# owensgroup/sparsify.me

Measured on AMD Instinct MI355X. Metric: effective GF/s (2:4 spmma vs dense gemm) on ResNet-50 layer shapes, higher is better.
Workload: dtype f16

## Files before the change

sparsify.me_amd/csrc/spmma_f16_fused.hip:

```cpp
#include "select24.h"
#include "spmma_args.h"

namespace sm {

constexpr int MAXG = 8;
struct FusedArgs {
  const half_t* A[MAXG];
  const half_t* B[MAXG];
  half_t* C[MAXG];
  size_t sA, sB, sC;
  int Mrows, N, K, lda;
  int batch, tiles_m, tiles_n;
  int ngroup;
  float alpha, beta;
  const half_t* const* dAp;
  const half_t* const* dBp;
  half_t* const* dCp;
};

struct FusedArgsEpi : FusedArgs {
  EpiArgs e;
};
template <bool EPI> struct FusedArgsSel { typedef FusedArgs type; };
template <> struct FusedArgsSel<true> { typedef FusedArgsEpi type; };
// ... 800 lines not shown
      for (; kt0 + 2 * PF < nkt; kt0 += PF) {
#pragma unroll
        for (int u = 0; u < PF; ++u) step(kt0 + u, ra[(u + 1) % PF], true, true);
      }
    } else {
#pragma unroll
      for (int s = 0; s < PF; ++s)
        if (s < nkt) load_a(s, ra[s]);
      write_stage(0, ra[0]);
      if (PF < nkt) load_a(PF, ra[0]);
    }
    for (; kt0 < nkt; kt0 += PF) {
#pragma unroll
      for (int u = 0; u < PF; ++u) {
        const int kt = kt0 + u;
        if (kt < nkt) step(kt, ra[(u + 1) % PF], kt + 1 < nkt, kt + 1 + PF < nkt);
      }
    }
  } else {
    int cb = 0;
    BTileDma<BN, NBW> bd;
    int nb = NSB - 1;
    if (NLB == 0) {
      bd.setup(p.B[grp] + (size_t)b * p.sB, p.N, n0, wave, lane, BRING);
#pragma unroll
      for (int s = 0; s < NSB - 1; ++s)
        if (s < nkt) bd.issue(smem, s, (unsigned)(s * SB));
    }
    for (int kt = 0; kt < nkt; ++kt) {
      if (NLB == 0) {
        if (kt + NSB - 2 < nkt) wait_dma_and_barrier<(NSB - 2) * B_WI>();
        else wait_dma_and_barrier<0>();
        if (kt + NSB - 1 < nkt) {
          bd.issue(smem, kt + NSB - 1, (unsigned)(nb * SB));
          nb = nb + 1 == NSB ? 0 : nb + 1;
        }
      } else {
        wait_dma_and_barrier<0>();
      }
      const char* As = smem + (kt & 1) * ASTG;
      const char* Ms = As + SA;
      const char* Bs = smem + BRING + cb * SB;
      smfmac_stage<FM, FN, BF>(As, Ms, Bs, wm * TM, wn * TN, lane, acc);
      cb = cb + 1 == NSB ? 0 : cb + 1;
    }
  }
  __syncthreads();

  if constexpr (EPI) store_c_tile_epi<BM, BN, FM, FN, 64 * NW, BF>(smem, C, p.e.R + (size_t)b * p.e.sR, p.e, eb, acc, wave < (unsigned)NC, wm * TM, wn * TN, m0, n0, p.Mrows, p.N, p.alpha, p.beta, tid);
  else store_c_tile<BM, BN, FM, FN, 64 * NW, BF>(smem, C, acc, wave < (unsigned)NC, wm * TM, wn * TN, m0, n0, p.Mrows, p.N, p.alpha, p.beta, tid);
}

template <int BN, int WM, int WN, int NLB, int PF, int NSB, bool BF = false, bool ANT = true, bool EPI = false>
static int launch_fused_wide(const typename FusedArgsSel<EPI>::type& a0, hipStream_t st) {
  typename FusedArgsSel<EPI>::type a = a0;
  a.tiles_m = (a.Mrows + 127) / 128;
  a.tiles_n = (a.N + BN - 1) / BN;
  const size_t nwg = (size_t)a.tiles_m * a.tiles_n * a.batch * a.ngroup;
  constexpr size_t lds_main = 2 * (size_t)128 * 72 + (size_t)NSB * 64 * BN * 2;
  constexpr size_t lds_epi = (size_t)128 * (BN * 2 + 16);
  constexpr size_t lds = lds_main > lds_epi ? lds_main : lds_epi;
  return launch_grid<&spmma_f16_fused_wide_kernel<BN, WM, WN, NLB, PF, NSB, BF, ANT, EPI>>(nwg, 64 * (WM * WN + 4 + NLB), lds, lds, st, "sm_spmma_fused_f16",
                                                                                          "spmma_f16_fused_wide_kernel", a);
}

template <int BN, int WM, int WN, int NLB, int PF, int NSB, bool BF = false>
__global__ __launch_bounds__(64 * (WM * WN + 4 + NLB)) void spmma_f16_fused_widep_kernel(const FusedArgs p, const unsigned total) {
  constexpr int BM = 128, NLA = 4, NC = WM * WN;
  static_assert(NLB > 0 && PF >= 1 && PF <= 3 && NSB >= 2 && NSB <= 4, "pipeline depths");
  constexpr int TM = BM / WM, TN = BN / WN, FM = TM / 16, FN = TN / 16;
  static_assert(TN == 128 && TM == 32, "epilogue patch geometry");
  constexpr int SA = BM * 64, SM_ = BM * 8, ASTG = SA + SM_, SB = 64 * BN * 2;
  constexpr int BRING = 2 * ASTG;
  constexpr int B_N = BN / 8, B_WI = B_N / NLB;
  static_assert(B_N % NLB == 0 && (NSB - 2) * B_WI <= 63, "B tile vs loader waves");
  constexpr int WPITCH = 64 * 2 + 8, WPATCH = TM * WPITCH;
  constexpr int CPATCH = BRING + NSB * SB;
  extern __shared__ __attribute__((aligned(16))) char smem[];

  const unsigned tid = threadIdx.x, lane = tid & 63u;
  const unsigned wave = __builtin_amdgcn_readfirstlane(tid >> 6);
  const unsigned tiles = (unsigned)p.tiles_m * (unsigned)p.tiles_n;
  const int nkt = p.K / 64;
  const unsigned my_tiles = (total - blockIdx.x + gridDim.x - 1u) / gridDim.x;
  const int S = (int)my_tiles * nkt;

  struct Tile {
    unsigned grp, b;
    int m0, n0;
  };
  auto tile_of = [&](unsigned j) {
    Tile t;
    const unsigned lid = xcd_remap(blockIdx.x + j * gridDim.x, total);
    const unsigned gb = lid / tiles, trem = lid - gb * tiles;
    t.grp = gb / (unsigned)p.batch;
    t.b = gb - t.grp * (unsigned)p.batch;
    const unsigned tile_m = trem / (unsigned)p.tiles_n, tile_n = trem - tile_m * (unsigned)p.tiles_n;
    t.m0 = (int)tile_m * BM;
    t.n0 = (int)tile_n * BN;
    return t;
  };

  if (wave >= (unsigned)(NC + NLA)) {
    BTileDma<BN, NLB> bd;
    unsigned ij = 0;
    int ikt = 0, nb = 0;
    {
      const Tile t = tile_of(0);
      bd.setup(p.B[t.grp] + (size_t)t.b * p.sB, p.N, t.n0, wave - (NC + NLA), lane, BRING);
    }
    auto issue = [&]() {
      bd.issue(smem, ikt, (unsigned)(nb * SB));
      nb = nb + 1 == NSB ? 0 : nb + 1;
      if (++ikt == nkt) {
        ikt = 0;
        if (++ij < my_tiles) {
          const Tile t = tile_of(ij);
          bd.setup(p.B[t.grp] + (size_t)t.b * p.sB, p.N, t.n0, wave - (NC + NLA), lane, BRING);
        }
      }
    };
#pragma unroll
    for (int s = 0; s < NSB - 1; ++s)
      if (s < S) issue();
    for (int g = 0; g < S; ++g) {
      if (g + NSB - 2 < S) wait_dma_and_barrier<(NSB - 2) * B_WI>();
      else wait_dma_and_barrier<0>();
      if (g + NSB - 1 < S) issue();
    }
  } else if (wave >= (unsigned)NC) {
    const unsigned lw = wave - NC;
    const unsigned c8 = lane & 7u;
    const half_t* a_src[4];
    unsigned a_val_off[4], a_meta_off[4];
#pragma unroll
    for (int i = 0; i < 4; ++i) {
      const unsigned row = 8u * (4u * lw + i) + (lane >> 3);
      a_val_off[i] = row * 64u + 16u * ((c8 >> 1) ^ a64_swz(row)) + 8u * (c8 & 1u);
      a_meta_off[i] = SA + row * 8u + c8;
    }
    const int mlast = p.Mrows - 1;
    auto point_at = [&](unsigned j) {
      const Tile t = tile_of(j);
      const half_t* A = p.A[t.grp] + (size_t)t.b * p.sA;
#pragma unroll
      for (int i = 0; i < 4; ++i) {
        const unsigned row = 8u * (4u * lw + i) + (lane >> 3);
        int gr = t.m0 + (int)row;
        gr = gr < mlast ? gr : mlast;
        a_src[i] = A + (size_t)gr * p.lda + 8u * c8;
      }
    };
    point_at(0);
    unsigned lj = 0;
    int lkt = 0;
    u4 ra[PF][4];
    auto load_a = [&](u4 (&dst)[4]) {
#pragma unroll
      for (int i = 0; i < 4; ++i) dst[i] = __builtin_nontemporal_load(reinterpret_cast<const u4*>(a_src[i] + (size_t)lkt * 64));
      __builtin_amdgcn_sched_barrier(0);
      if (++lkt == nkt) {
        lkt = 0;
        if (++lj < my_tiles) point_at(lj);
      }
    };
    auto write_stage = [&](int g, const u4 (&src)[4]) {
      char* sb = smem + (g & 1) * ASTG;
#pragma unroll
      for (int i = 0; i < 4; ++i) {
        uint32_t k0, k1, n0, n1;
        strip_select_f16(src[i][0], src[i][1], k0, n0);
        strip_select_f16(src[i][2], src[i][3], k1, n1);
        *reinterpret_cast<u2*>(sb + a_val_off[i]) = u2{k0, k1};
        *reinterpret_cast<unsigned char*>(sb + a_meta_off[i]) = (unsigned char)(n0 | (n1 << 4));
      }
    };
    auto step = [&](int g, u4 (&rr)[4], bool write, bool load) {
      asm volatile("s_waitcnt lgkmcnt(0)\n\ts_barrier" ::: "memory");
      __builtin_amdgcn_sched_barrier(0);
      if (write) write_stage(g + 1, rr);
      if (load) load_a(rr);
      __builtin_amdgcn_sched_barrier(0);
    };
    int g0 = 0;
    if (S > 2 * PF) {
#pragma unroll
      for (int s = 0; s < PF; ++s) load_a(ra[s]);
      write_stage(0, ra[0]);
      load_a(ra[0]);
      for (; g0 + 2 * PF < S; g0 += PF) {
#pragma unroll
        for (int u = 0; u < PF; ++u) step(g0 + u, ra[(u + 1) % PF], true, true);
      }
    } else {
#pragma unroll
      for (int s = 0; s < PF; ++s)
        if (s < S) load_a(ra[s]);
      write_stage(0, ra[0]);
      if (PF < S) load_a(ra[0]);
    }
    for (; g0 < S; g0 += PF) {
#pragma unroll
      for (int u = 0; u < PF; ++u) {
        const int g = g0 + u;
        if (g < S) step(g, ra[(u + 1) % PF], g + 1 < S, g + 1 + PF < S);
      }
    }
  } else {
    const unsigned g4 = lane >> 4, r = lane & 15u;
    const unsigned wm = wave / WN, wn = wave % WN;
    char* const patch = smem + CPATCH + wave * WPATCH;
    f4 acc[FM][FN];
#pragma unroll
    for (int i = 0; i < FM; ++i)
#pragma unroll
      for (int j = 0; j < FN; ++j) acc[i][j] = f4{0.f, 0.f, 0.f, 0.f};
    int cb = 0, kt = 0;
    unsigned cj = 0;
    Tile t = tile_of(0);
    for (int g = 0; g < S; ++g) {
      asm volatile("s_barrier" ::: "memory");
      const char* As = smem + (g & 1) * ASTG;
      smfmac_stage<FM, FN, BF>(As, As + SA, smem + BRING + cb * SB, wm * TM, wn * TN, lane, acc);
      cb = cb + 1 == NSB ? 0 : cb + 1;
      if (++kt == nkt) {
        half_t* C = p.C[t.grp] + (size_t)t.b * p.sC;
        const bool c_vec = (reinterpret_cast<uintptr_t>(C) & 15u) == 0 && (p.N % 8 == 0);
        if (p.beta == 0.0f && c_vec) {
#pragma unroll
          for (int h = 0; h < 2; ++h) {
#pragma unroll
            for (int i = 0; i < FM; ++i)
#pragma unroll
              for (int j = 0; j < FN / 2; ++j) {
                const unsigned lr = i * 16 + 4u * g4, lc = j * 16 + r;
#pragma unroll
                for (int q = 0; q < 4; ++q)
                  *reinterpret_cast<half_t*>(patch + (lr + q) * WPITCH + lc * 2) = to_elt<BF>(p.alpha * acc[i][h * (FN / 2) + j][q]);
              }
            asm volatile("s_waitcnt lgkmcnt(0)" ::: "memory");
            const int gc = t.n0 + (int)(wn * TN) + 64 * h + 8 * (int)(lane & 7u);
#pragma unroll
            for (int s8 = 0; s8 < TM / 8; ++s8) {
              const unsigned lr = 8u * s8 + (lane >> 3);
              const int gr = t.m0 + (int)(wm * TM + lr);
              if (gr < p.Mrows && gc < p.N) {
                const u2 lo = *reinterpret_cast<const u2*>(patch + lr * WPITCH + 16u * (lane & 7u));
                const u2 hi = *reinterpret_cast<const u2*>(patch + lr * WPITCH + 16u * (lane & 7u) + 8u);
                __builtin_nontemporal_store(u4{lo[0], lo[1], hi[0], hi[1]}, reinterpret_cast<u4*>(C + (size_t)gr * p.N + gc));
              }
            }
            asm volatile("s_waitcnt lgkmcnt(0)" ::: "memory");
          }
        } else {
#pragma unroll
          for (int i = 0; i < FM; ++i)
#pragma unroll
            for (int j = 0; j < FN; ++j) {
              const int gc = t.n0 + (int)(wn * TN + j * 16 + r);
              if (gc >= p.N) continue;
#pragma unroll
              for (int q = 0; q < 4; ++q) {
                const int gr = t.m0 + (int)(wm * TM + i * 16 + 4u * g4) + q;
                if (gr >= p.Mrows) continue;
                half_t* dst = C + (size_t)gr * p.N + gc;
                float v = p.alpha * acc[i][j][q];
                if (p.beta != 0.0f) v += p.beta * to_f32<BF>(*dst);
                *dst = to_elt<BF>(v);
              }
            }
        }
#pragma unroll
        for (int i = 0; i < FM; ++i)
#pragma unroll
          for (int j = 0; j < FN; ++j) acc[i][j] = f4{0.f, 0.f, 0.f, 0.f};
        kt = 0;
        if (++cj < my_tiles) t = tile_of(cj);
      }
    }
  }
}

template <int BN, int WM, int WN, int NLB, int PF, int NSB, bool BF = false>
static int launch_fused_widep(const FusedArgs& a0, hipStream_t st) {
  FusedArgs a = a0;
  a.tiles_m = (a.Mrows + 127) / 128;
  a.tiles_n = (a.N + BN - 1) / BN;
  const size_t nt = (size_t)a.tiles_m * a.tiles_n * a.batch * a.ngroup;
  if (nt == 0) return SM_STATUS_SUCCESS;
  if (nt > 0x7fffffffu) {
    set_error("sm_spmma_fused_f16: grid too large");
    return SM_STATUS_NOT_SUPPORTED;
  }
  constexpr size_t lds = 2 * (size_t)128 * 72 + (size_t)NSB * 64 * BN * 2 + (size_t)(WM * WN) * 32 * (64 * 2 + 8);
  static_assert(lds > 64 * 1024 && lds <= 160 * 1024, "LDS budget of the persistent wide kernel (always opted in)");
  size_t cus = (size_t)device_cu_count();
  cus -= cus % 8;
  if (cus == 0) cus = 8;
  return launch_grid<&spmma_f16_fused_widep_kernel<BN, WM, WN, NLB, PF, NSB, BF>>(nt <= cus ? nt : cus, 64 * (WM * WN + 4 + NLB), lds, lds, st, "sm_spmma_fused_f16",
                                                                                 "spmma_f16_fused_widep_kernel", a, (unsigned)nt);
}

constexpr int astat_waves_per_simd(int nwaves) { return nwaves == 16 ? 4 : (2 * nwaves + 3) / 4; }
template <int NSB, bool BF = false, int NLA = 4, int NLB = 4, int PR = 32>
__global__ __launch_bounds__(64 * (8 + NLA + NLB), astat_waves_per_simd(8 + NLA + NLB)) void spmma_f16_fused_astat_kernel(const FusedArgs p, int nsplit, int tiles_per_split) {
  constexpr int BM = 128, BN = 128, WM = 4, WN = 2, NC = 8;
  constexpr int NW = NC + NLA + NLB, RPL = (16 + NW - 1) / NW, KTM = 8 / RPL;
  static_assert(NW <= 16 && RPL <= 2 && (PR == 32 || PR == 16 || PR == 8), "launch bounds, phase-1 registers, patch passes");
  constexpr int TM = BM / WM, TN = BN / WN, FM = TM / 16, FN = TN / 16;
  constexpr int SA = BM * 64, SM_ = BM * 8, ASTG = SA + SM_, SB = 64 * BN * 2;
  constexpr int B_N = BN / 8, B_WI = B_N / NLB;
  static_assert((NSB - 2) * B_WI <= 63, "vmcnt range");
  constexpr int WPITCH = TN * 2 + 8, WPATCH = PR * WPITCH;
  static_assert(NLA != 0 || (PR == 16 ? 3 : 4) * ASTG + NSB * SB + NC * WPATCH <= 80 * 1024, "two workgroups per CU: 80 KiB each (astat_pair_lds_bytes)");
  extern __shared__ __attribute__((aligned(16))) char smem[];

  const unsigned tid = threadIdx.x, lane = tid & 63u;
  const unsigned wave = __builtin_amdgcn_readfirstlane(tid >> 6);
  const int nkt = p.K / 64;
  const unsigned per_batch = (unsigned)p.tiles_m * (unsigned)nsplit;
  const unsigned lid = xcd_remap(blockIdx.x, gridDim.x);
  const unsigned gb = lid / per_batch, trem = lid - gb * per_batch;
  const unsigned grp = gb / (unsigned)p.batch, b = gb - grp * (unsigned)p.batch;
  const unsigned tile_m = trem / (unsigned)nsplit, split = trem - tile_m * (unsigned)nsplit;
  const int m0 = (int)tile_m * BM;
  const int nt0 = (int)split * tiles_per_split;
  const int nt1 = nt0 + tiles_per_split < p.tiles_n ? nt0 + tiles_per_split : p.tiles_n;
  const int T = (nt1 - nt0) * nkt;
  char* const Bring = smem + nkt * ASTG;
  char* const Cpatch = Bring + NSB * SB;
  half_t* C = p.C[grp] + (size_t)b * p.sC;

  const bool is_b = wave >= (unsigned)(NC + NLA);
  const unsigned lwb = is_b ? wave - (NC + NLA) : 0u;
  const char* Bb = reinterpret_cast<const char*>(p.B[grp] + (size_t)b * p.sB);
  unsigned b_kr[B_WI], b_col[B_WI], b_dst[B_WI];
  auto b_lanes = [&](unsigned ln) {
#pragma unroll
    for (int i = 0; i < B_WI; ++i) {
      const unsigned j = lwb + (unsigned)NLB * i, panel = j >> 3, grp = j & 7u, kr = 8u * grp + (ln >> 3);
      b_kr[i] = kr;
      b_col[i] = 64u * panel + 8u * ((ln & 7u) ^ b_swz(kr));
      b_dst[i] = panel * 8192u + grp * 1024u;
    }
  };
  b_lanes(lane);
  const size_t row_bytes = (size_t)p.N * 2;
  int i_nt = nt0, i_kt = 0, i_buf = 0;
  auto issue_b = [&]() {
#pragma unroll
    for (int i = 0; i < B_WI; ++i) {
      int gc = i_nt * BN + (int)b_col[i];
      gc = gc <= p.N - 8 ? gc : p.N - 8;
      const char* src = Bb + (size_t)(i_kt * 64 + (int)b_kr[i]) * row_bytes + (size_t)gc * 2;
      __builtin_amdgcn_global_load_lds((gptr_t*)src, (lptr_t*)(Bring + i_buf * SB + b_dst[i]), 16, 0, 0);
    }
    i_buf = i_buf + 1 == NSB ? 0 : i_buf + 1;
    if (++i_kt == nkt) { i_kt = 0; ++i_nt; }
  };
  if (is_b) {
#pragma unroll
    for (int s = 0; s < NSB - 1; ++s)
      if (s < T) issue_b();
  }

  {
    const half_t* A = p.A[grp] + (size_t)b * p.sA;
    const unsigned c8 = lane & 7u;
    u4 ra[RPL][KTM];
#pragma unroll
    for (int h = 0; h < RPL; ++h) {
      const unsigned rg = wave + (unsigned)(NW * h);
      if (RPL == 1 || rg < 16u) {
        int gr = m0 + (int)(8u * rg + (lane >> 3));
        gr = gr < p.Mrows - 1 ? gr : p.Mrows - 1;
        const half_t* a_src = A + (size_t)gr * p.lda + 8u * c8;
#pragma unroll
        for (int s = 0; s < KTM; ++s)
          if (s < nkt) ra[h][s] = __builtin_nontemporal_load(reinterpret_cast<const u4*>(a_src + (size_t)s * 64));
      }
    }
#pragma unroll
    for (int h = 0; h < RPL; ++h) {
      const unsigned rg = wave + (unsigned)(NW * h);
      if (RPL == 1 || rg < 16u) {
        const unsigned row = 8u * rg + (lane >> 3);
        const unsigned a_val_off = row * 64u + 16u * ((c8 >> 1) ^ a64_swz(row)) + 8u * (c8 & 1u);
        const unsigned a_meta_off = SA + row * 8u + c8;
#pragma unroll
        for (int s = 0; s < KTM; ++s)
          if (s < nkt) {
            uint32_t k0, k1, n0, n1;
            strip_select_f16(ra[h][s][0], ra[h][s][1], k0, n0);
            strip_select_f16(ra[h][s][2], ra[h][s][3], k1, n1);
            char* sb = smem + s * ASTG;
            *reinterpret_cast<u2*>(sb + a_val_off) = u2{k0, k1};
            *reinterpret_cast<unsigned char*>(sb + a_meta_off) = (unsigned char)(n0 | (n1 << 4));
          }
      }
    }
  }
  if constexpr (RPL > 1) {
    unsigned ln = lane;
    asm volatile("" : "+v"(ln));
    b_lanes(ln);
  }
  __syncthreads();
  if (wave >= (unsigned)NC && !is_b) {
    for (int it = 0; it < T; ++it) asm volatile("s_barrier" ::: "memory");
    return;
  }

  if (is_b) {
    for (int it = 0; it < T; ++it) {
      if (it + NSB - 2 < T) wait_dma_and_barrier<(NSB - 2) * B_WI>();
      else wait_dma_and_barrier<0>();
      if (it + NSB - 1 < T) issue_b();
    }
  } else {
    const unsigned g = lane >> 4, r = lane & 15u;
    const unsigned wm = wave / WN, wn = wave % WN;
    char* const patch = Cpatch + wave * WPATCH;
    f4 acc[FM][FN];
#pragma unroll
    for (int i = 0; i < FM; ++i)
#pragma unroll
      for (int j = 0; j < FN; ++j) acc[i][j] = f4{0.f, 0.f, 0.f, 0.f};
    int cb = 0, kt = 0, nt = nt0;
    for (int it = 0; it < T; ++it) {
      asm volatile("s_barrier" ::: "memory");
      const char* As = smem + kt * ASTG;
      const char* Ms = As + SA;
      const char* Bs = Bring + cb * SB;
      smfmac_stage<FM, FN, BF>(As, Ms, Bs, wm * TM, wn * TN, lane, acc);
      cb = cb + 1 == NSB ? 0 : cb + 1;
      if (++kt == nkt) {
        if constexpr (PR == TM) {
          const int gc = nt * BN + (int)(wn * TN) + 8 * (int)(lane & 7u);
#pragma unroll
          for (int i = 0; i < FM; ++i)
#pragma unroll
            for (int j = 0; j < FN; ++j) {
              const unsigned lr = i * 16 + 4u * g, lc = j * 16 + r;
#pragma unroll
              for (int q = 0; q < 4; ++q) {
                *reinterpret_cast<half_t*>(patch + (lr + q) * WPITCH + lc * 2) = to_elt<BF>(p.alpha * acc[i][j][q]);
                acc[i][j][q] = 0.f;
              }
            }
          asm volatile("s_waitcnt lgkmcnt(0)" ::: "memory");
#pragma unroll
          for (int s = 0; s < TM / 8; ++s) {
            const unsigned lr = 8u * s + (lane >> 3);
            const int gr = m0 + (int)(wm * TM + lr);
            if (gr < p.Mrows && gc < p.N) {
              const u2 lo = *reinterpret_cast<const u2*>(patch + lr * WPITCH + 16u * (lane & 7u));
              const u2 hi = *reinterpret_cast<const u2*>(patch + lr * WPITCH + 16u * (lane & 7u) + 8u);
              __builtin_nontemporal_store(u4{lo[0], lo[1], hi[0], hi[1]}, reinterpret_cast<u4*>(C + (size_t)gr * p.N + gc));
            }
          }
        } else {
          unsigned le = lane;
          asm volatile("" : "+v"(le));
          const int gce = nt * BN + (int)(wn * TN) + 8 * (int)(le & 7u);
#pragma unroll
          for (int i = 0; i < FM; ++i)
#pragma unroll
            for (int h = 0; h < 16 / PR; ++h) {
              if (PR == 16 || (g >> 1) == (unsigned)h) {
#pragma unroll
                for (int j = 0; j < FN; ++j) {
                  const unsigned lr = 4u * (g & (unsigned)(PR / 4 - 1)), lc = j * 16 + r;
#pragma unroll
                  for (int q = 0; q < 4; ++q) *reinterpret_cast<half_t*>(patch + (lr + q) * WPITCH + lc * 2) = to_elt<BF>(p.alpha * acc[i][j][q]);
                }
              }
              asm volatile("s_waitcnt lgkmcnt(0)" ::: "memory");
#pragma unroll
              for (int s = 0; s < PR / 8; ++s) {
                const unsigned lr = 8u * s + (le >> 3);
                const int gr = m0 + (int)(wm * TM + i * 16 + h * PR + lr);
                if (gr < p.Mrows && gce < p.N) {
                  const u2 lo = *reinterpret_cast<const u2*>(patch + lr * WPITCH + 16u * (le & 7u));
                  const u2 hi = *reinterpret_cast<const u2*>(patch + lr * WPITCH + 16u * (le & 7u) + 8u);
                  __builtin_nontemporal_store(u4{lo[0], lo[1], hi[0], hi[1]}, reinterpret_cast<u4*>(C + (size_t)gr * p.N + gce));
                }
              }
            }
#pragma unroll
          for (int i = 0; i < FM; ++i)
#pragma unroll
            for (int j = 0; j < FN; ++j) acc[i][j] = f4{0.f, 0.f, 0.f, 0.f};
        }
        kt = 0;
        ++nt;
      }
    }
  }
}


static size_t astat_nsplit(size_t panels, size_t tiles_n, size_t cus) {
  size_t nsplit = 1;
  while (panels * nsplit * 4 < 3 * cus && (tiles_n + 2 * nsplit - 1) / (2 * nsplit) >= 2) nsplit *= 2;
  return nsplit;
}
static size_t astat_lds_bytes(int nkt, int nsb) { return (size_t)nkt * (128 * 72) + (size_t)nsb * 64 * 128 * 2 + 8 * 32 * (64 * 2 + 8); }

constexpr int ASTAT_PAIR_NLB = 4;
static bool astat_pair_takes(int nkt, size_t nwg, int nsplit, size_t cus) { return nkt <= 3 || (nkt == 4 && nsplit == 1 && 4 * nwg >= 7 * cus); }
static size_t astat_pair_lds_bytes(int nkt) { return (size_t)nkt * (128 * 72) + (size_t)2 * 64 * 128 * 2 + 8 * (nkt <= 3 ? 16 : 8) * (64 * 2 + 8); }
static_assert(3 * (128 * 72) + 2 * 64 * 128 * 2 + 8 * 16 * 136 == 77824 && 4 * (128 * 72) + 2 * 64 * 128 * 2 + 8 * 8 * 136 == 78336, "LDS of the two-per-CU kernels");

template <auto KERNEL>
static bool two_resident_per_cu(unsigned threads, size_t lds, hipStream_t st) {
  static std::atomic<signed char> known[256];
  int dev = 0;
  if (hipGetDevice(&dev) != hipSuccess || dev < 0 || dev >= 256) return false;
  signed char k = known[dev].load(std::memory_order_relaxed);
  if (k == 0) {
    hipStreamCaptureStatus cs = hipStreamCaptureStatusNone;
    if (hipStreamIsCapturing(st, &cs) != hipSuccess) {
      (void)hipGetLastError();
      return false;
    }
    if (cs != hipStreamCaptureStatusNone) return false;
    static LdsOptIn optin;
    int nb = 0;
    if (ensure_dyn_lds(optin, reinterpret_cast<const void*>(KERNEL), lds, "spmma_f16_fused_astat_kernel") != SM_STATUS_SUCCESS ||
        hipOccupancyMaxActiveBlocksPerMultiprocessor(&nb, KERNEL, (int)threads, lds) != hipSuccess) {
      (void)hipGetLastError();
      nb = 0;
    }
    k = nb >= 2 ? 1 : -1;
    known[dev].store(k, std::memory_order_relaxed);
  }
  return k > 0;
}

template <bool BF = false>
static int launch_fused_astat(const FusedArgs& a0, hipStream_t st) {
  FusedArgs a = a0;
  a.tiles_m = (a.Mrows + 127) / 128;
  a.tiles_n = (a.N + 127) / 128;
  const size_t panels = (size_t)a.tiles_m * a.batch * a.ngroup;
  const size_t cus = (size_t)device_cu_count();
  int nsplit = (int)astat_nsplit(panels, (size_t)a.tiles_n, cus);
  int tps = (a.tiles_n + nsplit - 1) / nsplit;
  nsplit = (a.tiles_n + tps - 1) / tps;
  const size_t nwg = panels * nsplit;
  const int nkt = a.K / 64;
  if (astat_pair_takes(nkt, nwg, nsplit, cus)) {
    constexpr unsigned threads = 64 * (8 + ASTAT_PAIR_NLB);
    const size_t lds = astat_pair_lds_bytes(nkt);
    if (nkt <= 3) {
      constexpr auto kernel = &spmma_f16_fused_astat_kernel<2, BF, 0, ASTAT_PAIR_NLB, 16>;
      if (two_resident_per_cu<kernel>(threads, 80 * 1024, st))
        return launch_grid<kernel>(nwg, threads, 80 * 1024, lds, st, "sm_spmma_fused_f16", "spmma_f16_fused_astat_kernel", a, nsplit, tps);
    } else {
      constexpr auto kernel = &spmma_f16_fused_astat_kernel<2, BF, 0, ASTAT_PAIR_NLB, 8>;
      if (two_resident_per_cu<kernel>(threads, 80 * 1024, st))
        return launch_grid<kernel>(nwg, threads, 80 * 1024, lds, st, "sm_spmma_fused_f16", "spmma_f16_fused_astat_kernel", a, nsplit, tps);
    }
  }
  constexpr int NSB = 3;
  return launch_grid<&spmma_f16_fused_astat_kernel<NSB, BF>>(nwg, 64 * 16, 160 * 1024, astat_lds_bytes(a.K / 64, NSB), st, "sm_spmma_fused_f16",
                                                            "spmma_f16_fused_astat_kernel", a, nsplit, tps);
}

}

using namespace sm;

static bool span_lds_fits(size_t n, size_t k) { return ((size_t)128 * k * 2 + 1152) + ((k + 63) / 64 * 64) * (n <= 64 ? 64 : 128) * 2 <= 160 * 1024; }
static bool span_form_takes(size_t m, size_t n, size_t k, size_t lda, size_t batch, size_t strideA, size_t strideB, size_t strideC, bool all_aligned, bool c_aligned) {
  return (k % 64 != 0 || lda % 8 != 0) && lda == k && n % 8 == 0 && n <= 128 && all_aligned && c_aligned && (batch == 1 || (strideB == 0 && strideA == m * lda && strideC == m * n)) &&
         (m * batch * k * 2) % 16 == 0 && m * batch <= 0x7fffffffull && k <= 0x7fffffffull && span_lds_fits(n, k);
}
static bool stage_forms_take(size_t n, size_t k, size_t lda, size_t strideA, size_t strideB, bool all_aligned) {
  return !(k % 64 != 0 || lda % 8 != 0 || strideA % 8 != 0 || n % 8 != 0 || strideB % 8 != 0 || !all_aligned);
}
static bool dims_fit_int(size_t m, size_t n, size_t k, size_t lda, size_t batch) {
  return !(m * batch > 0x7fffffffull || n > 0x7fffffffull || k > 0x7fffffffull || lda > 0x7fffffffull);
}

struct FusedCall {
  size_t m, n, k, lda, batch, count, sA, sB, sC;
  float beta;
  bool a_aligned, b_aligned, c_aligned;
  bool ws, ws_aligned;
  size_t ws_bytes;
  bool epi, r_aligned;
  size_t sR;
};
struct FusedPick {
  int form;
  bool stacked;
  const char* why;
};

static FusedPick fused_form(const FusedCall& c, size_t cus) {
  const size_t m = c.m, n = c.n, k = c.k, lda = c.lda, batch = c.batch;
  if (c.count == 0 || m == 0 || n == 0 || batch == 0) return {SM_FUSED_FORM_EMPTY, false, nullptr};
  const bool all_aligned = c.a_aligned && c.b_aligned;
  const bool contiguous = c.sB == 0 && c.sA == m * lda && c.sC == m * n;
  if (n < 8 && k <= 64 && lda == k && (batch == 1 || contiguous)) {
    if (c.epi) return {SM_FUSED_FORM_NOT_TAKEN, false, "sm_spmma_fused_{f16,bf16}_ex: the thin form (n < 8) takes no epilogue"};
    if (thin_form_takes(c.count, m * batch, n, k) && c.a_aligned) return {SM_FUSED_FORM_THIN, true, nullptr};
  }
  const bool r_follows = !c.epi || c.beta == 0.0f || (c.r_aligned && (batch == 1 || c.sR == m * n));
  if (span_form_takes(m, n, k, lda, batch, c.sA, c.sB, c.sC, all_aligned, c.c_aligned && r_follows)) return {SM_FUSED_FORM_SPAN, true, nullptr};
  if (!stage_forms_take(n, k, lda, c.sA, c.sB, all_aligned))
    return {SM_FUSED_FORM_NOT_TAKEN, false, "sm_spmma_fused_{f16,bf16}: needs k % 64 == 0, n % 8 == 0 and 16-byte aligned rows (use the staged path)"};
  if (c.count > 1 && !c.c_aligned)
    return {SM_FUSED_FORM_NOT_TAKEN, false, "sm_spmma_fused_{f16,bf16}_grouped: needs 16-byte aligned C operands"};
  if (!dims_fit_int(m, n, k, lda, batch)) return {SM_FUSED_FORM_NOT_TAKEN, false, "sm_spmma_fused_{f16,bf16}: dimension exceeds 2^31-1"};
  const bool stacked = batch > 1 && contiguous && (!c.epi || c.beta == 0.0f || c.sR == m * n);
  const size_t rows = stacked ? m * batch : m, nb = (stacked ? 1 : batch) * c.count;
  const bool astat_store = n > 256 && k <= 512 && c.beta == 0.0f && c.c_aligned && (c.sC % 8 == 0);
  if (c.ws) {
    SkPlan pl;
    if (sk_takes(rows, nb, n, k, astat_store, cus, pl) && c.ws_bytes >= sk_workspace_bytes((size_t)pl.slots * ((n + 255) / 256), 256) && c.ws_aligned &&
        !sk_launch_limits((rows + 255) / 256 * nb, n, k, lda, cus))
      return {SM_FUSED_FORM_STREAMK, stacked, nullptr};
  }
  auto round_eff = [](size_t tiles, size_t cus_) { const size_t r = (tiles + cus_ - 1) / cus_; return r ? (double)tiles / (double)(r * cus_) : 1.0; };
  if (n > 128 && k > 64) {
    const size_t t_big = (rows + 255) / 256 * ((n + 255) / 256) * nb, t_wide = (rows + 127) / 128 * ((n + 255) / 256) * nb;
    bool big = round_eff(t_big, cus) >= round_eff(t_wide, cus);
    if (!c.epi && astat_store) {
      const size_t panels = (rows + 127) / 128 * nb;
      big = round_eff(t_big, cus) > round_eff(panels * astat_nsplit(panels, (n + 127) / 128, cus), cus) + 0.1;
    }
    if (big) return {SM_FUSED_FORM_BIG, stacked, nullptr};
  }
  if (n <= 128 || (n <= 256 && k <= 64)) {
    if (n <= 64) return {SM_FUSED_FORM_DIRECT64, stacked, nullptr};
    return {n > 128 || k < 512 ? SM_FUSED_FORM_DIRECT128 : SM_FUSED_FORM_DIRECT128_NT, stacked, nullptr};
  }
  if (!c.epi && astat_store && astat_lds_bytes((int)(k / 64), 3) <= 160 * 1024) return {SM_FUSED_FORM_ASTAT, stacked, nullptr};
  if (k <= 1024 && !c.epi) return {SM_FUSED_FORM_WIDEP, stacked, nullptr};
  return {n > 256 ? SM_FUSED_FORM_WIDE : SM_FUSED_FORM_WIDE_NT, stacked, nullptr};
}

static bool fused_form_is_exact(int form) { return form != SM_FUSED_FORM_NOT_TAKEN && form != SM_FUSED_FORM_EMPTY && form != SM_FUSED_FORM_THIN; }

bool sm::spmma_fused16_takes_exact(const void* A, const void* B, const void* C, size_t m, size_t n, size_t k, size_t lda, size_t batch, size_t strideA, size_t strideB,
                                   size_t strideC) {
  if (!A || !B || !C || lda < k) return false;
  const FusedCall c = {m, n, k, lda, batch, 1, strideA, strideB, strideC, 0.0f, aligned16(A), aligned16(B), aligned16(C), false, false, 0, false, false, 0};
  return fused_form_is_exact(fused_form(c, 256).form);
}

extern "C" int sm_spmma_fused_form(size_t m, size_t n, size_t k, size_t lda, size_t batch, size_t count, size_t strideA, size_t strideB, size_t strideC,
                                   float beta, unsigned flags, size_t cus, int* form) {
  constexpr unsigned known = SM_FUSED_FLAG_A_ALIGNED | SM_FUSED_FLAG_B_ALIGNED | SM_FUSED_FLAG_C_ALIGNED | SM_FUSED_FLAG_WORKSPACE | SM_FUSED_FLAG_EPILOGUE;
  if (!form || lda < k || count > (size_t)MAXG || (flags & ~known) || ((flags & SM_FUSED_FLAG_WORKSPACE) && (flags & SM_FUSED_FLAG_EPILOGUE))) {
    set_error("sm_spmma_fused_form: invalid argument");
    return SM_STATUS_INVALID_VALUE;
  }
  const bool c_al = (flags & SM_FUSED_FLAG_C_ALIGNED) != 0, ws = (flags & SM_FUSED_FLAG_WORKSPACE) != 0;
  const FusedCall c = {m, n, k, lda, batch, count, strideA, strideB, strideC, beta, (flags & SM_FUSED_FLAG_A_ALIGNED) != 0, (flags & SM_FUSED_FLAG_B_ALIGNED) != 0, c_al,
                       ws, ws, ws ? ~(size_t)0 : 0, (flags & SM_FUSED_FLAG_EPILOGUE) != 0, c_al, strideC};
  *form = fused_form(c, cus ? cus : (size_t)device_cu_count()).form;
  return SM_STATUS_SUCCESS;
}

template <bool BF>
static int spmma_fused16(size_t ngroup, const void* const* Ag, const void* const* Bg, void* const* Cg, size_t m, size_t n, size_t k, size_t lda,
                         size_t batch, size_t strideA, size_t strideB, size_t strideC, float alpha, float beta,
                         sm_stream_t stream, void* workspace = nullptr, size_t workspace_bytes = 0, const EpiArgs* epi = nullptr) {
#define SM_LAUNCH(fn, ...) (epi ? fn<__VA_ARGS__, true>(ae, st) : fn<__VA_ARGS__, false>(a, st))
  if (ngroup == 0) return SM_STATUS_SUCCESS;
  if (!Ag || !Bg || !Cg || lda < k || ngroup > (size_t)MAXG) {
    set_error("sm_spmma_fused_{f16,bf16}: invalid argument");
    return SM_STATUS_INVALID_VALUE;
  }
  FusedCall c = {m, n, k, lda, batch, ngroup, strideA, strideB, strideC, beta, true, true, true, workspace != nullptr, aligned16(workspace), workspace_bytes,
                 epi != nullptr, epi && aligned16(epi->R), epi ? epi->sR : 0};
  for (size_t g = 0; g < ngroup; ++g) {
    if (!Ag[g] || !Bg[g] || !Cg[g]) {
      set_error("sm_spmma_fused_{f16,bf16}: invalid argument (null operand)");
      return SM_STATUS_INVALID_VALUE;
    }
    c.a_aligned = c.a_aligned && aligned16(Ag[g]);
    c.b_aligned = c.b_aligned && aligned16(Bg[g]);
    c.c_aligned = c.c_aligned && aligned16(Cg[g]);
  }
  const FusedPick pick = fused_form(c, (size_t)device_cu_count());
  hipStream_t st = (hipStream_t)stream;
  FusedArgs a = {};
  for (size_t g = 0; g < (size_t)MAXG; ++g) {
    const size_t s_ = g < ngroup ? g : 0;
    a.A[g] = (const half_t*)Ag[s_]; a.B[g] = (const half_t*)Bg[s_]; a.C[g] = (half_t*)Cg[s_];
  }
  a.ngroup = (int)ngroup;
  a.N = (int)n; a.K = (int)k; a.lda = (int)lda;
  a.alpha = alpha; a.beta = beta;
  if (pick.stacked) {
    a.Mrows = (int)(m * batch);
    a.batch = 1;
  } else {
    a.Mrows = (int)m;
    a.batch = (int)batch;
  }
  if (pick.form != SM_FUSED_FORM_SPAN) { a.sA = strideA; a.sB = strideB; a.sC = strideC; }
  FusedArgsEpi ae = {};
  static_cast<FusedArgs&>(ae) = a;
  if (epi) ae.e = *epi;
  switch (pick.form) {
    case SM_FUSED_FORM_EMPTY: return SM_STATUS_SUCCESS;
    case SM_FUSED_FORM_NOT_TAKEN:
      set_error("%s", pick.why);
      return SM_STATUS_NOT_SUPPORTED;
    case SM_FUSED_FORM_THIN: return spmma_fused_thin(BF, (int)ngroup, Ag, Bg, Cg, m * batch, n, k, alpha, beta, st);
    case SM_FUSED_FORM_SPAN: return n <= 64 ? SM_LAUNCH(launch_fused_span, 64, BF, false) : SM_LAUNCH(launch_fused_span, 128, BF, false);
    case SM_FUSED_FORM_STREAMK:
      return n <= 256 ? launch_fused_sk<256, BF, true>(a, workspace, workspace_bytes, st) : launch_fused_sk<256, BF, false>(a, workspace, workspace_bytes, st);
    case SM_FUSED_FORM_BIG: return n <= 256 ? SM_LAUNCH(launch_fused_big, 256, BF, 3, 2, true, false) : SM_LAUNCH(launch_fused_big, 256, BF, 3, 2, false, false);
    case SM_FUSED_FORM_DIRECT64: return SM_LAUNCH(launch_fused_direct, 64, 2, BF, 128, 4, true, false);
    case SM_FUSED_FORM_DIRECT128: return SM_LAUNCH(launch_fused_direct, 128, 2, BF, 128, 4, false, false);
    case SM_FUSED_FORM_DIRECT128_NT: return SM_LAUNCH(launch_fused_direct, 128, 2, BF, 128, 4, true, false);
    case SM_FUSED_FORM_ASTAT: return launch_fused_astat<BF>(a, st);
    case SM_FUSED_FORM_WIDEP: return launch_fused_widep<256, 4, 2, 4, 2, 3, BF>(a, st);
    case SM_FUSED_FORM_WIDE: return SM_LAUNCH(launch_fused_wide, 256, 4, 2, 4, 2, 3, BF, false);
    case SM_FUSED_FORM_WIDE_NT: return SM_LAUNCH(launch_fused_wide, 256, 4, 2, 4, 2, 3, BF, true);
  }
  set_error("sm_spmma_fused_{f16,bf16}: internal error (unknown form)");
  return SM_STATUS_LAUNCH_FAILED;
#undef SM_LAUNCH
}

extern "C" int sm_spmma_fused_f16(const void* A, const void* B, void* C, size_t m, size_t n, size_t k, size_t lda,
                                  size_t batch, size_t strideA, size_t strideB, size_t strideC, float alpha, float beta,
                                  sm_stream_t stream) {
  return spmma_fused16<false>(1, &A, &B, &C, m, n, k, lda, batch, strideA, strideB, strideC, alpha, beta, stream);
}
extern "C" int sm_spmma_fused_bf16(const void* A, const void* B, void* C, size_t m, size_t n, size_t k, size_t lda,
                                   size_t batch, size_t strideA, size_t strideB, size_t strideC, float alpha, float beta,
                                   sm_stream_t stream) {
  return spmma_fused16<true>(1, &A, &B, &C, m, n, k, lda, batch, strideA, strideB, strideC, alpha, beta, stream);
}

template <bool BF>
static int spmma_fused16_ex(const void* A, const void* B, void* D, size_t m, size_t n, size_t k, size_t lda, size_t batch, size_t strideA, size_t strideB,
                            size_t strideD, float alpha, float beta, const sm_epilogue_t* ep, sm_stream_t stream) {
  EpiArgs e;
  bool plain;
  if (const int rc = epilogue_args(ep, D, strideD, m, beta, e, &plain, "sm_spmma_fused_{f16,bf16}_ex")) return rc;
  return spmma_fused16<BF>(1, &A, &B, &D, m, n, k, lda, batch, strideA, strideB, strideD, alpha, beta, stream, nullptr, 0, plain ? nullptr : &e);
}
extern "C" int sm_spmma_fused_f16_ex(const void* A, const void* B, void* D, size_t m, size_t n, size_t k, size_t lda, size_t batch,
                                     size_t strideA, size_t strideB, size_t strideD, float alpha, float beta, const sm_epilogue_t* epilogue,
                                     sm_stream_t stream) {
  return spmma_fused16_ex<false>(A, B, D, m, n, k, lda, batch, strideA, strideB, strideD, alpha, beta, epilogue, stream);
}
extern "C" int sm_spmma_fused_bf16_ex(const void* A, const void* B, void* D, size_t m, size_t n, size_t k, size_t lda, size_t batch,
                                      size_t strideA, size_t strideB, size_t strideD, float alpha, float beta, const sm_epilogue_t* epilogue,
                                      sm_stream_t stream) {
  return spmma_fused16_ex<true>(A, B, D, m, n, k, lda, batch, strideA, strideB, strideD, alpha, beta, epilogue, stream);
}

extern "C" int sm_spmma_fused_workspace_size(size_t* bytes) {
  if (!bytes) {
    set_error("sm_spmma_fused_workspace_size: invalid argument");
    return SM_STATUS_INVALID_VALUE;
  }
  *bytes = sk_workspace_bytes((size_t)device_cu_count(), 256);
  return SM_STATUS_SUCCESS;
}
extern "C" int sm_spmma_fused_workspace_state(const void* workspace, int* state, sm_stream_t stream) {
  if (!workspace || !state) {
    set_error("sm_spmma_fused_workspace_state: invalid argument");
    return SM_STATUS_INVALID_VALUE;
  }
  unsigned h[1024];
  hipStream_t st = (hipStream_t)stream;
  if (hipMemcpyAsync(h, workspace, sizeof(h), hipMemcpyDeviceToHost, st) != hipSuccess || hipStreamSynchronize(st) != hipSuccess)
    return check_launch("sm_spmma_fused_workspace_state");
  bool dirty = false;
  for (int i = 0; i < 1023; ++i) dirty = dirty || h[i] != 0u;
  *state = h[1023] != 0u ? 1 : (dirty ? 2 : 0);
  return SM_STATUS_SUCCESS;
}
extern "C" int sm_spmma_fused_streamk_plan(size_t rows, size_t n, size_t k, size_t problems, int* takes, unsigned* plan) {
  if (!takes || !plan) {
    set_error("sm_spmma_fused_streamk_plan: invalid argument");
    return SM_STATUS_INVALID_VALUE;
  }
  SkPlan pl = {};
  *takes = sk_takes(rows, problems, n, k, n > 256 && k <= 512, (size_t)device_cu_count(), pl) ? 1 : 0;
  unsigned* o = plan;
  *o++ = pl.tg; *o++ = pl.wg; *o++ = pl.groups_full; *o++ = pl.tgl; *o++ = pl.wgl; *o++ = pl.slots; *o++ = pl.units;
  for (int i = 0; i < 9; ++i) *o++ = pl.cut[i];
  for (int i = 0; i < 9; ++i) *o++ = pl.cutl[i];
  return SM_STATUS_SUCCESS;
}
extern "C" int sm_spmma_fused_f16_ws(const void* A, const void* B, void* C, size_t m, size_t n, size_t k, size_t lda, size_t batch, size_t strideA,
                                     size_t strideB, size_t strideC, float alpha, float beta, void* workspace, size_t workspace_bytes, sm_stream_t stream) {
  return spmma_fused16<false>(1, &A, &B, &C, m, n, k, lda, batch, strideA, strideB, strideC, alpha, beta, stream, workspace, workspace_bytes);
}
extern "C" int sm_spmma_fused_bf16_ws(const void* A, const void* B, void* C, size_t m, size_t n, size_t k, size_t lda, size_t batch, size_t strideA,
                                      size_t strideB, size_t strideC, float alpha, float beta, void* workspace, size_t workspace_bytes, sm_stream_t stream) {
  return spmma_fused16<true>(1, &A, &B, &C, m, n, k, lda, batch, strideA, strideB, strideC, alpha, beta, stream, workspace, workspace_bytes);
}

template <bool BF>
static int dense_twin16(const DenseTwinCall& c, hipStream_t st) {
  const size_t n = (size_t)c.N, k = (size_t)c.K;
  const bool tables = c.Ap != nullptr;
  if (tables != (c.Bp != nullptr) || tables != (c.Cp != nullptr)) return SM_STATUS_NOT_SUPPORTED;
  if (c.N % 8 != 0 || c.N < 8 || (!tables && (!aligned16(c.A) || !aligned16(c.B) || !aligned16(c.C)))) return SM_STATUS_NOT_SUPPORTED;
  FusedArgs a = {};
  for (int g = 0; g < MAXG; ++g) { a.A[g] = c.A; a.B[g] = c.B; a.C[g] = c.C; }
  a.dAp = c.Ap; a.dBp = c.Bp; a.dCp = c.Cp;
  a.ngroup = 1;
  a.sA = c.sA; a.sB = c.sB; a.sC = c.sC;
  a.Mrows = c.M; a.N = c.N; a.K = c.K; a.lda = c.lda;
  a.batch = c.batch; a.alpha = c.alpha; a.beta = c.beta;
  if (k % 64 != 0 || c.lda % 8 != 0) {
    if (c.lda != c.K || n > 128 || ((size_t)c.M * k * 2) % 16 != 0 || (c.batch > 1 && !tables)) return SM_STATUS_NOT_SUPPORTED;
    if (!span_lds_fits(n, k)) return SM_STATUS_NOT_SUPPORTED;
    a.ngroup = c.batch;
    a.batch = 1;
    if (!tables) a.ngroup = 1;
    return n <= 64 ? launch_fused_span<64, BF, true>(a, st) : launch_fused_span<128, BF, true>(a, st);
  }
  if (c.sA % 8 != 0 || c.sB % 8 != 0) return SM_STATUS_NOT_SUPPORTED;
  if (c.workspace && n > 128 && n <= 256 && k >= 2048) {
    SkPlan pl;
    if (sk_takes((size_t)c.M, (size_t)c.batch, n, k, false, (size_t)device_cu_count(), pl) && c.workspace_bytes >= sk_workspace_bytes((size_t)pl.slots * ((n + 255) / 256), 256) &&
        aligned16(c.workspace))
      return launch_fused_sk<256, BF, true, true>(a, c.workspace, c.workspace_bytes, st);
  }
  if (n <= 128) return SM_STATUS_NOT_SUPPORTED;
  if (k <= 64) return SM_STATUS_NOT_SUPPORTED;
  if (((size_t)c.M + 255) / 256 * 256 * 100 > (size_t)c.M * 115) return SM_STATUS_NOT_SUPPORTED;
  if (!(n <= 256 && k >= 2048)) return SM_STATUS_NOT_SUPPORTED;
  return launch_fused_big<256, BF, 3, 2, true, true>(a, st);
}

int sm::gemm_dense_twin(const DenseTwinCall& c, hipStream_t st) { return c.bf ? dense_twin16<true>(c, st) : dense_twin16<false>(c, st); }

template <bool BF>
static int spmma_fused16_grouped(size_t count, const void* const* A, const void* const* B, void* const* C, size_t m, size_t n, size_t k,
                                 size_t lda, size_t batch, size_t strideA, size_t strideB, size_t strideC, float alpha, float beta,
                                 sm_stream_t stream, void* workspace = nullptr, size_t workspace_bytes = 0) {
  if (count && (!A || !B || !C)) {
    set_error("sm_spmma_fused_{f16,bf16}_grouped: invalid argument");
    return SM_STATUS_INVALID_VALUE;
  }
  for (size_t i = 0; i < count; i += (size_t)MAXG) {
    const size_t ng = count - i < (size_t)MAXG ? count - i : (size_t)MAXG;
    if (const int rc = spmma_fused16<BF>(ng, A + i, B + i, C + i, m, n, k, lda, batch, strideA, strideB, strideC, alpha, beta, stream, workspace, workspace_bytes)) return rc;
  }
  return SM_STATUS_SUCCESS;
}
extern "C" int sm_spmma_fused_f16_grouped(size_t count, const void* const* A, const void* const* B, void* const* C, size_t m, size_t n,
                                          size_t k, size_t lda, size_t batch, size_t strideA, size_t strideB, size_t strideC,
                                          float alpha, float beta, sm_stream_t stream) {
  return spmma_fused16_grouped<false>(count, A, B, C, m, n, k, lda, batch, strideA, strideB, strideC, alpha, beta, stream);
}
extern "C" int sm_spmma_fused_bf16_grouped(size_t count, const void* const* A, const void* const* B, void* const* C, size_t m, size_t n,
// ... 15 lines not shown
```

Baseline: 597,600.

## Use four consumer waves in the two-per-CU astat kernel for k=256

```diff
diff --git a/sparsify.me_amd/csrc/spmma_f16_fused.hip b/sparsify.me_amd/csrc/spmma_f16_fused.hip
--- a/sparsify.me_amd/csrc/spmma_f16_fused.hip
+++ b/sparsify.me_amd/csrc/spmma_f16_fused.hip
@@ -1126,17 +1126,19 @@
 }
 
 constexpr int astat_waves_per_simd(int nwaves) { return nwaves == 16 ? 4 : (2 * nwaves + 3) / 4; }
-template <int NSB, bool BF = false, int NLA = 4, int NLB = 4, int PR = 32>
-__global__ __launch_bounds__(64 * (8 + NLA + NLB), astat_waves_per_simd(8 + NLA + NLB)) void spmma_f16_fused_astat_kernel(const FusedArgs p, int nsplit, int tiles_per_split) {
-  constexpr int BM = 128, BN = 128, WM = 4, WN = 2, NC = 8;
+template <int NSB, bool BF = false, int NLA = 4, int NLB = 4, int PR = 32, int NCW = 8>
+__global__ __launch_bounds__(64 * (NCW + NLA + NLB), astat_waves_per_simd(NCW + NLA + NLB)) void spmma_f16_fused_astat_kernel(const FusedArgs p, int nsplit, int tiles_per_split) {
+  constexpr int BM = 128, BN = 128, WM = NCW / 2, WN = 2, NC = NCW;
   constexpr int NW = NC + NLA + NLB, RPL = (16 + NW - 1) / NW, KTM = 8 / RPL;
-  static_assert(NW <= 16 && RPL <= 2 && (PR == 32 || PR == 16 || PR == 8), "launch bounds, phase-1 registers, patch passes");
+  static_assert((NCW == 8 || NCW == 4) && NW >= 8 && NW <= 16 && RPL <= 2, "consumer grid, launch bounds, phase-1 registers");
   constexpr int TM = BM / WM, TN = BN / WN, FM = TM / 16, FN = TN / 16;
+  static_assert(PR == TM || PR == 16, "the write-out goes in one piece of PR == TM rows or per 16-row fragment");
+  static_assert(NCW == 8 || (NLA == 0 && NW == 8 && astat_waves_per_simd(NW) == 4), "4 consumers: 8 waves, 4 per SIMD with two workgroups on the CU");
   constexpr int SA = BM * 64, SM_ = BM * 8, ASTG = SA + SM_, SB = 64 * BN * 2;
   constexpr int B_N = BN / 8, B_WI = B_N / NLB;
   static_assert((NSB - 2) * B_WI <= 63, "vmcnt range");
   constexpr int WPITCH = TN * 2 + 8, WPATCH = PR * WPITCH;
-  static_assert(NLA != 0 || (PR == 16 ? 3 : 4) * ASTG + NSB * SB + NC * WPATCH <= 80 * 1024, "two workgroups per CU: 80 KiB each (astat_pair_lds_bytes)");
+  static_assert(NLA != 0 || (NCW == 8 ? 3 : 4) * ASTG + NSB * SB + NC * WPATCH <= 80 * 1024, "two workgroups per CU: 80 KiB each, k <= 192 / 256 (astat_pair_lds_bytes)");
   extern __shared__ __attribute__((aligned(16))) char smem[];
 
   const unsigned tid = threadIdx.x, lane = tid & 63u;
@@ -1288,29 +1290,25 @@
           asm volatile("" : "+v"(le));
           const int gce = nt * BN + (int)(wn * TN) + 8 * (int)(le & 7u);
 #pragma unroll
-          for (int i = 0; i < FM; ++i)
-#pragma unroll
-            for (int h = 0; h < 16 / PR; ++h) {
-              if (PR == 16 || (g >> 1) == (unsigned)h) {
-#pragma unroll
-                for (int j = 0; j < FN; ++j) {
-                  const unsigned lr = 4u * (g & (unsigned)(PR / 4 - 1)), lc = j * 16 + r;
-#pragma unroll
-                  for (int q = 0; q < 4; ++q) *reinterpret_cast<half_t*>(patch + (lr + q) * WPITCH + lc * 2) = to_elt<BF>(p.alpha * acc[i][j][q]);
-                }
-              }
-              asm volatile("s_waitcnt lgkmcnt(0)" ::: "memory");
-#pragma unroll
-              for (int s = 0; s < PR / 8; ++s) {
-                const unsigned lr = 8u * s + (le >> 3);
-                const int gr = m0 + (int)(wm * TM + i * 16 + h * PR + lr);
-                if (gr < p.Mrows && gce < p.N) {
-                  const u2 lo = *reinterpret_cast<const u2*>(patch + lr * WPITCH + 16u * (le & 7u));
-                  const u2 hi = *reinterpret_cast<const u2*>(patch + lr * WPITCH + 16u * (le & 7u) + 8u);
-                  __builtin_nontemporal_store(u4{lo[0], lo[1], hi[0], hi[1]}, reinterpret_cast<u4*>(C + (size_t)gr * p.N + gce));
-                }
+          for (int i = 0; i < FM; ++i) {
+#pragma unroll
+            for (int j = 0; j < FN; ++j) {
+              const unsigned lr = 4u * g, lc = j * 16 + r;
+#pragma unroll
+              for (int q = 0; q < 4; ++q) *reinterpret_cast<half_t*>(patch + (lr + q) * WPITCH + lc * 2) = to_elt<BF>(p.alpha * acc[i][j][q]);
+            }
+            asm volatile("s_waitcnt lgkmcnt(0)" ::: "memory");
+#pragma unroll
+            for (int s = 0; s < PR / 8; ++s) {
+              const unsigned lr = 8u * s + (le >> 3);
+              const int gr = m0 + (int)(wm * TM + i * 16 + lr);
+              if (gr < p.Mrows && gce < p.N) {
+                const u2 lo = *reinterpret_cast<const u2*>(patch + lr * WPITCH + 16u * (le & 7u));
+                const u2 hi = *reinterpret_cast<const u2*>(patch + lr * WPITCH + 16u * (le & 7u) + 8u);
+                __builtin_nontemporal_store(u4{lo[0], lo[1], hi[0], hi[1]}, reinterpret_cast<u4*>(C + (size_t)gr * p.N + gce));
               }
             }
+          }
 #pragma unroll
           for (int i = 0; i < FM; ++i)
 #pragma unroll
@@ -1332,9 +1330,10 @@
 static size_t astat_lds_bytes(int nkt, int nsb) { return (size_t)nkt * (128 * 72) + (size_t)nsb * 64 * 128 * 2 + 8 * 32 * (64 * 2 + 8); }
 
 constexpr int ASTAT_PAIR_NLB = 4;
-static bool astat_pair_takes(int nkt, size_t nwg, int nsplit, size_t cus) { return nkt <= 3 || (nkt == 4 && nsplit == 1 && 4 * nwg >= 7 * cus); }
-static size_t astat_pair_lds_bytes(int nkt) { return (size_t)nkt * (128 * 72) + (size_t)2 * 64 * 128 * 2 + 8 * (nkt <= 3 ? 16 : 8) * (64 * 2 + 8); }
-static_assert(3 * (128 * 72) + 2 * 64 * 128 * 2 + 8 * 16 * 136 == 77824 && 4 * (128 * 72) + 2 * 64 * 128 * 2 + 8 * 8 * 136 == 78336, "LDS of the two-per-CU kernels");
+static bool astat_pair_takes(int nkt, size_t nwg, size_t cus) { return nkt <= 3 || (nkt == 4 && nwg > cus); }
+static int astat_pair_consumers(int nkt) { return nkt == 4 ? 4 : 8; }
+static size_t astat_pair_lds_bytes(int nkt) { return (size_t)nkt * (128 * 72) + (size_t)2 * 64 * 128 * 2 + (size_t)astat_pair_consumers(nkt) * 16 * (64 * 2 + 8); }
+static_assert(3 * (128 * 72) + 2 * 64 * 128 * 2 + 8 * 16 * 136 == 77824 && 4 * (128 * 72) + 2 * 64 * 128 * 2 + 4 * 16 * 136 == 78336, "LDS of the two-per-CU kernels");
 
 template <auto KERNEL>
 static bool two_resident_per_cu(unsigned threads, size_t lds, hipStream_t st) {
@@ -1374,15 +1373,16 @@
   nsplit = (a.tiles_n + tps - 1) / tps;
   const size_t nwg = panels * nsplit;
   const int nkt = a.K / 64;
-  if (astat_pair_takes(nkt, nwg, nsplit, cus)) {
-    constexpr unsigned threads = 64 * (8 + ASTAT_PAIR_NLB);
+  if (astat_pair_takes(nkt, nwg, cus)) {
     const size_t lds = astat_pair_lds_bytes(nkt);
-    if (nkt <= 3) {
-      constexpr auto kernel = &spmma_f16_fused_astat_kernel<2, BF, 0, ASTAT_PAIR_NLB, 16>;
+    if (astat_pair_consumers(nkt) == 4) {
+      constexpr unsigned threads = 64 * (4 + ASTAT_PAIR_NLB);
+      constexpr auto kernel = &spmma_f16_fused_astat_kernel<2, BF, 0, ASTAT_PAIR_NLB, 16, 4>;
       if (two_resident_per_cu<kernel>(threads, 80 * 1024, st))
         return launch_grid<kernel>(nwg, threads, 80 * 1024, lds, st, "sm_spmma_fused_f16", "spmma_f16_fused_astat_kernel", a, nsplit, tps);
     } else {
-      constexpr auto kernel = &spmma_f16_fused_astat_kernel<2, BF, 0, ASTAT_PAIR_NLB, 8>;
+      constexpr unsigned threads = 64 * (8 + ASTAT_PAIR_NLB);
+      constexpr auto kernel = &spmma_f16_fused_astat_kernel<2, BF, 0, ASTAT_PAIR_NLB, 16>;
       if (two_resident_per_cu<kernel>(threads, 80 * 1024, st))
         return launch_grid<kernel>(nwg, threads, 80 * 1024, lds, st, "sm_spmma_fused_f16", "spmma_f16_fused_astat_kernel", a, nsplit, tps);
     }
```

New measurement: 602,400 (median of 6 runs). About the same (+0.8%).
